# Haian-Jin/TensoIR

Hardware: AMD Instinct MI355X
Metric: primary+secondary rays/sec at 4096 rays x 512 samples (higher is better)
Workload: dtype f32 io and field; decoders split-bf16 x3 (hi/lo operands, 3 MFMA products), fp32 accumulate; indirect light (secondary-ray records): fp16 shadow taps + fp16 single-product decoder, fp32 accumulate

## Files before the change

tensoir_amd/csrc/tir_common.hpp:

```cpp
#pragma once
#include <hip/hip_runtime.h>
#include <stdint.h>
#include <initializer_list>
#include <type_traits>
#include "tensoir_hip.h"

#define TIR_WAVE 64

#define TIR_CHECK_LAUNCH()                                   \
    do {                                                     \
        hipError_t e__ = hipGetLastError();                  \
        if (e__ != hipSuccess) return -(int)e__;             \
    } while (0)

static inline hipStream_t tir_stream(void* s) { return reinterpret_cast<hipStream_t>(s); }

static inline int tir_xcd_mapping(const TirField* f) { return f->tune_xcd_order == 1 ? 1 : 0; }

#include <mutex>
#include <set>
#include <utility>
static inline int tir_allow_dynamic_lds(const void* kernel, int bytes) {
    static std::mutex mu;
    static std::set<std::pair<const void*, int>> done;
// ... 622 lines not shown
    }
    __builtin_amdgcn_wave_barrier();
    constexpr int PER = 64 / C4;
    const int slot_in = lane / C4, c = lane % C4;
    for (int base = 0; base < n; base += PER) {
        const int slot = base + slot_in;
        float part = 0.0f;
        if (slot < n) part = density_chunk_rec<C4>(f, ll, wr + slot * TIR_TAPREC, c);
        if (C4 >= 2) part += dpp_f<0xB1, 0xf>(0.0f, part);
        if (C4 >= 4) part += dpp_f<0x4E, 0xf>(0.0f, part);
        if (C4 >= 8) part += dpp_f<0x141, 0xf>(0.0f, part);
        if (slot < n && c == 0) wl[slot * TIR_TAPREC] = part;
    }
    __builtin_amdgcn_wave_barrier();
    float sig = 0.0f;
    if (valid) sig = feature2density(f, wl[rank * TIR_TAPREC]);
    __builtin_amdgcn_wave_barrier();
    return sig;
}

__device__ __forceinline__ float wave_sigma(const TirField& f, bool valid, float x, float y, float z, float* wl) {
    switch (f.n_dcomp) {
        case 16: return wave_sigma_t<4>(f, valid, x, y, z, wl);
        case 8:  return wave_sigma_t<2>(f, valid, x, y, z, wl);
        case 32: return wave_sigma_t<8>(f, valid, x, y, z, wl);
        default: return wave_sigma_t<1>(f, valid, x, y, z, wl);
    }
}

__device__ __forceinline__ float exp_neg_fast(float x) { return __builtin_amdgcn_exp2f(x * -1.4426950408889634f); }

__device__ __forceinline__ bool sample_valid(const TirField& f, float px, float py, float pz, float& x, float& y, float& z) {
    x = norm_coord(px, f.aabb_min[0], f.inv_aabb[0]);
    y = norm_coord(py, f.aabb_min[1], f.inv_aabb[1]);
    z = norm_coord(pz, f.aabb_min[2], f.inv_aabb[2]);
    if (!in_bbox(f, px, py, pz)) return false;
    if (f.occ_nbr != nullptr && !occupancy_hit(f, px, py, pz)) return false;
    return true;
}

__device__ __forceinline__ void occ_t_range(const float (&occ_lo)[3], const float (&occ_hi)[3], const float (&o)[3], const float (&d)[3],
                                            float& t0, float& t1) {
    t0 = -INFINITY; t1 = INFINITY;
    if (!((occ_lo[0] < occ_hi[0]) & (occ_lo[1] < occ_hi[1]) & (occ_lo[2] < occ_hi[2]))) return;
#pragma unroll
    for (int a = 0; a < 3; ++a) {
        if (fabsf(d[a]) < 1e-20f) {
            if ((o[a] < occ_lo[a]) | (o[a] > occ_hi[a])) { t0 = INFINITY; t1 = -INFINITY; }
        } else {
            const float inv = __builtin_amdgcn_rcpf(d[a]);
            const float ta = (occ_lo[a] - o[a]) * inv, tb = (occ_hi[a] - o[a]) * inv;
            t0 = fmaxf(t0, fminf(ta, tb));
            t1 = fminf(t1, fmaxf(ta, tb));
        }
    }
    t0 -= 1e-4f; t1 += 1e-4f;
}

struct UDiv { unsigned d, m; };
__device__ __forceinline__ UDiv make_udiv(int d) { return UDiv{d > 1 ? (unsigned)d : 1u, d > 1 ? 0xFFFFFFFFu / (unsigned)d : 0u}; }
__device__ __forceinline__ unsigned udiv(unsigned x, const UDiv& u, unsigned& rem) {
    if (u.d == 1) { rem = 0; return x; }
    unsigned q = __umulhi(x, u.m), r = x - q * u.d;
    if (r >= u.d) { q += 1; r -= u.d; }
    rem = r;
    return q;
}

__device__ __forceinline__ float linear2srgb(float x) {
    x = fminf(fmaxf(x, 0.0f), 1.0f);
    float lin = x * 12.92f;
    float nonlin = 1.055f * powf(x + 1e-6f, 0.41666666666666667f) - 0.055f;
    return (x <= 0.0031308f) ? lin : nonlin;
}

struct RaySetup {
    float o[3], d[3];
    float t_min;
};

__device__ __forceinline__ RaySetup ray_setup(const TirField& f, const float* __restrict__ rays, int r) {
    RaySetup s;
    float tm = -INFINITY;
#pragma unroll
    for (int a = 0; a < 3; ++a) {
        s.o[a] = rays[6 * (size_t)r + a];
        s.d[a] = rays[6 * (size_t)r + 3 + a];
        float vec = (s.d[a] == 0.0f) ? 1e-6f : s.d[a];
        float ra = __fdiv_rn(sub_rn(f.aabb_max[a], s.o[a]), vec);
        float rb = __fdiv_rn(sub_rn(f.aabb_min[a], s.o[a]), vec);
        tm = fmaxf(tm, fminf(ra, rb));
    }
    s.t_min = fminf(fmaxf(tm, f.near_), f.far_);
    return s;
}

__device__ __forceinline__ float sample_z(const TirField& f, float t_min, int k, float jitter, bool has_jitter) {
    float rng = (float)k;
    if (has_jitter) rng = add_rn(rng, jitter);
    return add_rn(t_min, mul_rn(f.step_size, rng));
}



__device__ __forceinline__ void philox_round(uint32_t (&c)[4], uint32_t k0, uint32_t k1) {
    const uint64_t p0 = (uint64_t)0xD2511F53u * c[0], p1 = (uint64_t)0xCD9E8D57u * c[2];
    const uint32_t n0 = (uint32_t)(p1 >> 32) ^ c[1] ^ k0, n2 = (uint32_t)(p0 >> 32) ^ c[3] ^ k1;
    c[0] = n0; c[1] = (uint32_t)p1; c[2] = n2; c[3] = (uint32_t)p0;
}

__device__ __forceinline__ void jitter_normals(unsigned long long seed, unsigned long long offset, uint64_t idx, float (&nrm)[3]) {
    uint32_t c[4] = {(uint32_t)idx, (uint32_t)(idx >> 32), (uint32_t)offset, (uint32_t)(offset >> 32)};
    uint32_t k0 = (uint32_t)seed, k1 = (uint32_t)(seed >> 32);
#pragma unroll
    for (int r = 0; r < 10; ++r) { philox_round(c, k0, k1); k0 += 0x9E3779B9u; k1 += 0xBB67AE85u; }
    const float u0 = ((float)c[0] + 0.5f) * 2.3283064365386963e-10f, u1 = ((float)c[1] + 0.5f) * 2.3283064365386963e-10f;
    const float u2 = ((float)c[2] + 0.5f) * 2.3283064365386963e-10f, u3 = ((float)c[3] + 0.5f) * 2.3283064365386963e-10f;
    const float r0 = sqrtf(-2.0f * logf(fminf(u0, 0.99999994f))), r1 = sqrtf(-2.0f * logf(fminf(u2, 0.99999994f)));
    float s0, c0, s1, c1;
    sincospif(2.0f * u1, &s0, &c0);
    sincospif(2.0f * u3, &s1, &c1);
    nrm[0] = r0 * c0; nrm[1] = r0 * s0; nrm[2] = r1 * c1;
    (void)s1;
}

__device__ __forceinline__ void philox_uniform4(unsigned long long seed, unsigned long long offset, uint64_t idx, float (&u)[4]) {
    uint32_t c[4] = {(uint32_t)idx, (uint32_t)(idx >> 32), (uint32_t)offset, (uint32_t)(offset >> 32)};
    uint32_t k0 = (uint32_t)seed, k1 = (uint32_t)(seed >> 32);
#pragma unroll
    for (int r = 0; r < 10; ++r) { philox_round(c, k0, k1); k0 += 0x9E3779B9u; k1 += 0xBB67AE85u; }
#pragma unroll
    for (int q = 0; q < 4; ++q) u[q] = fminf(((float)c[q] + 0.5f) * 2.3283064365386963e-10f, 0.99999994f);
}

struct XcdRange { long long first, end, stride; };
__device__ __forceinline__ XcdRange xcd_range_at(long long n_items, int per, bool on, int bid, int nblk) {
    XcdRange r;
    if (!on || (nblk & 7) != 0) {
        r.first = (long long)bid * per; r.end = n_items; r.stride = (long long)nblk * per;
        return r;
    }
    const int xcd = bid & 7, local = bid >> 3, per_xcd = nblk >> 3;
    const long long chunk = (n_items + 7) / 8;
    const long long lo = chunk * xcd;
    r.first = lo + (long long)local * per;
    r.end = lo + chunk < n_items ? lo + chunk : n_items;
    r.stride = (long long)per_xcd * per;
    return r;
}
__device__ __forceinline__ XcdRange xcd_range(long long n_items, int per, bool on) {
    return xcd_range_at(n_items, per, on, (int)blockIdx.x, (int)gridDim.x);
}

}
```

tensoir_amd/csrc/tir_march.hip:

```cpp
#include "tir_common.hpp"

using namespace tir;

__device__ __forceinline__ void march_one_ray(const TirField& f, const float* __restrict__ rays, const float* __restrict__ ray_jitter,
                                              int B, int S, float t_stop, float* __restrict__ weight, float* __restrict__ acc_out,
                                              float* __restrict__ depth_out, float* __restrict__ tend_out,
                                              int32_t* __restrict__ app_count, unsigned long long* __restrict__ stats,
                                              float* __restrict__ sigma_out, float* __restrict__ viewdirs, bool coh, int ray, int lane) {
    RaySetup rs = ray_setup(f, rays, ray);
    if (viewdirs && lane < 3) viewdirs[3 * (size_t)ray + lane] = rays[6 * (size_t)ray + 3 + lane];

    const bool hj = ray_jitter != nullptr;
    const float jit = hj ? ray_jitter[ray] : 0.0f;

    __shared__ __attribute__((aligned(16))) float wl_all[4][256];
    float* wl = wl_all[threadIdx.x >> 6];
    float T = 1.0f;
    float acc = 0.0f, depth = 0.0f;
    int cnt = 0;
    int k0 = 0;
    unsigned n_gather = 0;
    for (; k0 < S; k0 += 64) {
        const int k = k0 + lane;
        float z = 0.0f, x = 0.f, y = 0.f, zz = 0.f;
        bool valid = false;
        if (k < S) {
            z = sample_z(f, rs.t_min, k, jit, hj);
            float px = add_rn(rs.o[0], mul_rn(rs.d[0], z));
            float py = add_rn(rs.o[1], mul_rn(rs.d[1], z));
            float pz = add_rn(rs.o[2], mul_rn(rs.d[2], z));
            valid = sample_valid(f, px, py, pz, x, y, zz);
        }
        const float sigma = wave_sigma(f, valid, x, y, zz, wl);
        float w = 0.0f, v = 1.0f;
        if (k < S) {
            float dist = (k + 1 < S) ? sub_rn(sample_z(f, rs.t_min, k + 1, jit, hj), z) : 0.0f;
            float alpha = 1.0f - expf(-sigma * mul_rn(dist, f.distance_scale));
            v = add_rn(sub_rn(1.0f, alpha), 1e-10f);
            w = alpha;
        }
        float incl = scan_prod<64>(v, lane);
        float excl = shift_up1<64>(incl, lane);
        w = w * (T * excl);
        if (k < S) weight[(size_t)ray * S + k] = w;
        if (sigma_out && k < S) sigma_out[(size_t)ray * S + k] = sigma;
        acc += w;
        depth = fmaf(w, z, depth);
        cnt += __popcll(__ballot(w > f.weight_thres));
        if (stats) n_gather += __popcll(__ballot(valid));
        T = T * __shfl(incl, 63, 64);
        if (T < t_stop) { k0 += 64; break; }
    }
    for (; k0 < S; k0 += 64) {
        const int k = k0 + lane;
        if (k < S) weight[(size_t)ray * S + k] = 0.0f;
        if (sigma_out && k < S) sigma_out[(size_t)ray * S + k] = 0.0f;
    }
    acc = group_sum<64>(acc);
    depth = group_sum<64>(depth);
    if (lane == 0) {
        acc_out[ray] = acc;
        depth_out[ray] = depth;
        if (tend_out) tend_out[ray] = T;
        if (coh) __hip_atomic_store(app_count + ray, cnt, __ATOMIC_RELAXED, __HIP_MEMORY_SCOPE_AGENT);
        else app_count[ray] = cnt;
        if (stats) atomicAdd(stats, (unsigned long long)n_gather);
    }
}


struct TirMarchExtras {
    float* viewdirs;
    int32_t* zero_words; int n_zero;
    int32_t* ticket; int32_t* offsets; int cap; int32_t* total_out;
};

__device__ __forceinline__ void block_exclusive_scan_capped(const int32_t* __restrict__ counts, int32_t* __restrict__ offsets,
                                                             int n, int cap, int32_t* __restrict__ total_out) {
    __shared__ int32_t wsum[4];
    __shared__ int32_t carry_s;
    const int tid = threadIdx.x, lane = tid & 63, wv = tid >> 6;
    if (tid == 0) carry_s = 0;
    __syncthreads();
    for (int base = 0; base < n; base += 256) {
        const int i = base + tid;
        const int32_t v = (i < n) ? __hip_atomic_load(counts + i, __ATOMIC_RELAXED, __HIP_MEMORY_SCOPE_AGENT) : 0;
        int32_t incl = v;
#pragma unroll
        for (int d = 1; d < 64; d <<= 1) {
            int32_t o = __shfl_up(incl, d, 64);
            if (lane >= d) incl += o;
        }
        if (lane == 63) wsum[wv] = incl;
        __syncthreads();
        int32_t woff = 0;
        for (int q = 0; q < wv; ++q) woff += wsum[q];
        const int32_t carry = carry_s;
        if (i < n) offsets[i] = min(carry + woff + incl - v, cap);
        __syncthreads();
        if (tid == 255) carry_s = carry + woff + incl;
        __syncthreads();
    }
    if (tid == 0) {
        offsets[n] = min(carry_s, cap);
        if (total_out) *total_out = carry_s;
    }
}

__global__ void __launch_bounds__(256)
k_march_primary(TirField f, const float* __restrict__ rays, const float* __restrict__ ray_jitter,
                int B, int S, float t_stop, float* __restrict__ weight, float* __restrict__ acc_out,
                float* __restrict__ depth_out, float* __restrict__ tend_out, int32_t* __restrict__ app_count,
                unsigned long long* __restrict__ stats, float* __restrict__ sigma_out, TirMarchExtras ex) {
    const int lane = threadIdx.x & 63;
    const int ray = blockIdx.x * (blockDim.x >> 6) + (threadIdx.x >> 6);
    if (ex.zero_words && blockIdx.x == 0 && threadIdx.x < ex.n_zero) ex.zero_words[threadIdx.x] = 0;
    if (ray < B) march_one_ray(f, rays, ray_jitter, B, S, t_stop, weight, acc_out, depth_out, tend_out, app_count, stats,
                               sigma_out, ex.viewdirs, ex.ticket != nullptr, ray, lane);
    if (!ex.ticket) return;
    __shared__ int s_last;
    asm volatile("s_waitcnt vmcnt(0)" ::: "memory");
    __syncthreads();
    if (threadIdx.x == 0) {
        const int t = __hip_atomic_fetch_add(ex.ticket, 1, __ATOMIC_RELAXED, __HIP_MEMORY_SCOPE_AGENT);
        s_last = (t == (int)gridDim.x - 1);
        if (s_last) __hip_atomic_store(ex.ticket, 0, __ATOMIC_RELAXED, __HIP_MEMORY_SCOPE_AGENT);
    }
    __syncthreads();
    if (s_last) block_exclusive_scan_capped(app_count, ex.offsets, B, ex.cap, ex.total_out);
}

extern "C" int tir_march_primary_fwd(const TirField* f, const float* rays, const float* ray_jitter,
                                     int32_t B, int32_t S, float t_stop, float* weight, float* acc,
                                     float* depth, float* t_end, int32_t* app_count,
                                     unsigned long long* stats, void* stream) {
    if (!f || B < 0 || S <= 0) return TIR_ERR_ARG;
    if (B == 0) return TIR_OK;
    if (!rays || !weight || !acc || !depth || !app_count) return TIR_ERR_ARG;
    if (!(f->n_dcomp == 4 || f->n_dcomp == 8 || f->n_dcomp == 16 || f->n_dcomp == 32)) return TIR_ERR_UNSUPPORTED;
    if (!tir_occ_index_ok(f) || !tir_plane_index_ok(f)) return TIR_ERR_UNSUPPORTED;
    hipLaunchKernelGGL(k_march_primary, dim3((B + 3) / 4), dim3(256), 0, tir_stream(stream), *f, rays,
                       ray_jitter, B, S, t_stop, weight, acc, depth, t_end, app_count, stats, (float*)nullptr, TirMarchExtras{});
    TIR_CHECK_LAUNCH();
    return TIR_OK;
}

extern "C" int tir_march_primary_fused_fwd(const TirField* f, const float* rays, const float* ray_jitter,
                                           int32_t B, int32_t S, float t_stop, float* weight, float* acc,
                                           float* depth, float* t_end, int32_t* app_count, unsigned long long* stats,
                                           float* viewdirs, int32_t* zero_words, int32_t n_zero, int32_t* ticket,
                                           int32_t* offsets, int32_t cap, int32_t* total, void* stream) {
    if (!f || B < 0 || S <= 0 || n_zero < 0 || n_zero > 256 || cap < 0) return TIR_ERR_ARG;
    if ((ticket == nullptr) != (offsets == nullptr)) return TIR_ERR_ARG;
    if (B == 0) return TIR_OK;
    if (!rays || !weight || !acc || !depth || !app_count) return TIR_ERR_ARG;
    if (!(f->n_dcomp == 4 || f->n_dcomp == 8 || f->n_dcomp == 16 || f->n_dcomp == 32)) return TIR_ERR_UNSUPPORTED;
    if (!tir_occ_index_ok(f) || !tir_plane_index_ok(f)) return TIR_ERR_UNSUPPORTED;
    TirMarchExtras ex{viewdirs, zero_words, n_zero, ticket, offsets, cap, total};
    hipLaunchKernelGGL(k_march_primary, dim3((B + 3) / 4), dim3(256), 0, tir_stream(stream), *f, rays,
                       ray_jitter, B, S, t_stop, weight, acc, depth, t_end, app_count, stats, (float*)nullptr, ex);
    TIR_CHECK_LAUNCH();
    return TIR_OK;
}

extern "C" int tir_march_primary_train_fwd(const TirField* f, const float* rays, const float* ray_jitter,
                                           int32_t B, int32_t S, float t_stop, float* weight, float* sigma,
                                           float* acc, float* depth, float* t_end, int32_t* app_count, void* stream) {
    if (!f || B < 0 || S <= 0) return TIR_ERR_ARG;
    if (B == 0) return TIR_OK;
    if (!rays || !weight || !sigma || !acc || !depth || !app_count) return TIR_ERR_ARG;
    if (!(f->n_dcomp == 4 || f->n_dcomp == 8 || f->n_dcomp == 16 || f->n_dcomp == 32)) return TIR_ERR_UNSUPPORTED;
    if (!tir_occ_index_ok(f) || !tir_plane_index_ok(f)) return TIR_ERR_UNSUPPORTED;
    hipLaunchKernelGGL(k_march_primary, dim3((B + 3) / 4), dim3(256), 0, tir_stream(stream), *f, rays,
                       ray_jitter, B, S, t_stop, weight, acc, depth, t_end, app_count,
                       (unsigned long long*)nullptr, sigma, TirMarchExtras{});
    TIR_CHECK_LAUNCH();
    return TIR_OK;
}

__global__ void __launch_bounds__(1024)
k_exclusive_scan(const int32_t* __restrict__ counts, int32_t* __restrict__ offsets, int n, int cap,
                 int32_t* __restrict__ total_out) {
    __shared__ int32_t wsum[16];
    __shared__ int32_t carry_s;
    const int tid = threadIdx.x, lane = tid & 63, wv = tid >> 6;
    if (tid == 0) carry_s = 0;
    __syncthreads();
    for (int base = 0; base < n; base += 1024) {
        int i = base + tid;
        int32_t v = (i < n) ? counts[i] : 0;
        int32_t incl = v;
#pragma unroll
        for (int d = 1; d < 64; d <<= 1) {
            int32_t o = __shfl_up(incl, d, 64);
            if (lane >= d) incl += o;
        }
        if (lane == 63) wsum[wv] = incl;
        __syncthreads();
        int32_t woff = 0;
        for (int q = 0; q < wv; ++q) woff += wsum[q];
        int32_t carry = carry_s;
        if (i < n) offsets[i] = min(carry + woff + incl - v, cap);
        __syncthreads();
        if (tid == 1023) carry_s = carry + woff + incl;
        __syncthreads();
    }
    if (tid == 0) {
        offsets[n] = min(carry_s, cap);
        if (total_out) *total_out = carry_s;
    }
}

extern "C" int tir_exclusive_scan(const int32_t* counts, int32_t* offsets, int32_t n, void* stream) {
    if (!offsets || n < 0 || (n > 0 && !counts)) return TIR_ERR_ARG;
    hipLaunchKernelGGL(k_exclusive_scan, dim3(1), dim3(1024), 0, tir_stream(stream), counts, offsets, n, 0x7fffffff,
                       (int32_t*)nullptr);
    TIR_CHECK_LAUNCH();
    return TIR_OK;
}

extern "C" int tir_exclusive_scan_capped(const int32_t* counts, int32_t* offsets, int32_t n, int32_t cap,
                                         int32_t* total, void* stream) {
    if (!offsets || n < 0 || cap < 0 || (n > 0 && !counts)) return TIR_ERR_ARG;
    hipLaunchKernelGGL(k_exclusive_scan, dim3(1), dim3(1024), 0, tir_stream(stream), counts, offsets, n, cap, total);
    TIR_CHECK_LAUNCH();
    return TIR_OK;
}

struct TirCheck4 { const int32_t* cnt[4]; int64_t cap[4]; int n; };

__global__ void k_record_check(TirCheck4 c, int64_t* __restrict__ state, int64_t* __restrict__ host_out) {
    if (threadIdx.x != 0 || blockIdx.x != 0) return;
    int64_t over = state[4];
    for (int i = 0; i < 4; ++i) {
        int64_t v = 0;
        if (i < c.n) {
            v = *c.cnt[i];
            if (v > c.cap[i]) over = 1;
            if (v > state[i]) state[i] = v;
        }
        host_out[i] = v;
        host_out[4 + i] = state[i];
    }
    state[4] = over;
    host_out[8] = over;
    __threadfence_system();
}

extern "C" int tir_record_check(const int32_t* const* counters, const int64_t* caps, int32_t n, int64_t* state,
                                int64_t* host_out, void* stream) {
    if (n < 0 || n > 4 || !state || !host_out || (n > 0 && (!counters || !caps))) return TIR_ERR_ARG;
// ... 581 lines not shown
        }
        __syncthreads();
        int32_t* const rec_ray = s_park.rec_ray;
        float* const rec_w = s_park.rec_w;
        float* const rec_xyz = s_park.rec_xyz;
#pragma unroll
        for (int g = 0; g < 4; ++g) {
            const int rl = g * NHW + hw;
            int base = s_base[rl];
            if (base < 0) continue;
            const int64_t ray = s_pid[rl];
            const float4 s0 = *reinterpret_cast<const float4*>(sh + 24 * g);
            const float2 s1 = *reinterpret_cast<const float2*>(sh + 24 * g + 4);
            const float o[3] = {s0.x, s0.y, s0.z}, d[3] = {s0.w, s1.x, s1.y};
#pragma unroll
            for (int st = 0; st < NSTEP; ++st) {
                const int k = st * 32 + hl;
                const float w = wreg[REC ? g : 0][REC ? st : 0];
                const bool keep = w > f.weight_thres;
                const unsigned hm = (unsigned)(__ballot(keep) >> half_shift);
                if (keep) {
                    const int slot = base + __popc(hm & ((1u << hl) - 1u));
                    const float z = zt[k];
                    rec_ray[slot] = (int32_t)ray;
                    rec_w[slot] = w;
#pragma unroll
                    for (int a = 0; a < 3; ++a) {
                        float p = add_rn(o[a], mul_rn(d[a], z));
                        rec_xyz[3 * (size_t)slot + a] = norm_coord(p, f.aabb_min[a], f.inv_aabb[a]);
                    }
                }
                base += __popc(hm);
            }
        }
    }
    if (stats && hl == 0 && n_gather) atomicAdd(s_park.stats, (unsigned long long)n_gather);
}

#define TIR_SEC_KERNEL_PARAMS                                                                                                  \
    TirField f, const float* __restrict__ origins, const int32_t* __restrict__ org_map, const float* __restrict__ dirs,       \
    const int32_t* __restrict__ dir_map, const uint8_t* __restrict__ active, int64_t n_rays, int n_dirs, int n_sample,        \
    const float* __restrict__ z_vals, float t_stop, float* __restrict__ vis, float* __restrict__ one_minus_acc,               \
    int32_t* __restrict__ rec_counter, int64_t rec_cap, int32_t* __restrict__ rec_ray, float* __restrict__ rec_w,             \
    float* __restrict__ rec_xyz, int32_t* __restrict__ ray_rec_off, int32_t* __restrict__ ray_rec_cnt,                        \
    unsigned long long* __restrict__ stats, int xcd_on, const int32_t* __restrict__ ray_ids, const int32_t* __restrict__ n_ids_dev
#define TIR_SEC_KERNEL_ARGS                                                                                                    \
    f, origins, org_map, dirs, dir_map, active, n_rays, n_dirs, n_sample, z_vals, t_stop, vis, one_minus_acc, rec_counter,    \
    rec_cap, rec_ray, rec_w, rec_xyz, ray_rec_off, ray_rec_cnt, stats, xcd_on, ray_ids, n_ids_dev

template <int C4, int NSTEP, int NT, bool REC>
__global__ void __launch_bounds__(NT, 4)
k_march_secondary_lds(TIR_SEC_KERNEL_PARAMS, int line_floats) {
    march_secondary_body<C4, NSTEP, NT, REC, false>(TIR_SEC_KERNEL_ARGS, line_floats);
}

#define TIR_DENSE_WAVES 6
template <int NSTEP, bool REC>
__global__ void __launch_bounds__(512, TIR_DENSE_WAVES)
k_march_secondary_dense(TIR_SEC_KERNEL_PARAMS) {
    march_secondary_body<1, NSTEP, 512, REC, true>(TIR_SEC_KERNEL_ARGS, 0);
}


extern "C" int tir_march_secondary_fwd(const TirField* f, const float* origins, const int32_t* org_map,
                                       const float* dirs, const int32_t* dir_map, const uint8_t* active,
                                       int64_t n_rays, int32_t n_dirs, int32_t n_sample, const float* z_vals,
                                       float t_stop, float* vis, float* one_minus_acc,
                                       int32_t* rec_counter, int64_t rec_cap, int32_t* rec_ray,
                                       float* rec_w, float* rec_xyz, int32_t* ray_rec_off,
                                       int32_t* ray_rec_cnt, unsigned long long* stats, void* stream) {
    return tir_march_secondary_ids_fwd(f, origins, org_map, dirs, dir_map, active, n_rays, n_dirs, n_sample, z_vals, t_stop,
                                       vis, one_minus_acc, rec_counter, rec_cap, rec_ray, rec_w, rec_xyz, ray_rec_off,
                                       ray_rec_cnt, stats, nullptr, nullptr, stream);
}

extern "C" int tir_march_secondary_ids_fwd(const TirField* f, const float* origins, const int32_t* org_map,
                                           const float* dirs, const int32_t* dir_map, const uint8_t* active,
                                           int64_t n_rays, int32_t n_dirs, int32_t n_sample, const float* z_vals,
                                           float t_stop, float* vis, float* one_minus_acc,
                                           int32_t* rec_counter, int64_t rec_cap, int32_t* rec_ray,
                                           float* rec_w, float* rec_xyz, int32_t* ray_rec_off,
                                           int32_t* ray_rec_cnt, unsigned long long* stats, const int32_t* ray_ids,
                                           const int32_t* n_ids_dev, void* stream) {
    if (!f || n_rays < 0 || n_sample <= 0) return TIR_ERR_ARG;
    if ((ray_ids == nullptr) != (n_ids_dev == nullptr)) return TIR_ERR_ARG;
    if (n_sample > TIR_SEC_MAX_SAMPLES) return TIR_ERR_UNSUPPORTED;
    if (n_rays == 0) return TIR_OK;
    if (!origins || !dirs || !z_vals) return TIR_ERR_ARG;
    if (rec_counter && (!rec_ray || !rec_w || !rec_xyz || !ray_rec_off || !ray_rec_cnt || rec_cap < 0)) return TIR_ERR_ARG;
    if (n_rays >= (int64_t)1 << 31) return TIR_ERR_UNSUPPORTED;
    if (!(f->n_dcomp == 4 || f->n_dcomp == 8 || f->n_dcomp == 16 || f->n_dcomp == 32)) return TIR_ERR_UNSUPPORTED;
    if (!tir_occ_index_ok(f) || !tir_plane_index_ok(f)) return TIR_ERR_UNSUPPORTED;
    const int xcd_on = tir_xcd_mapping(f);
    if (tir_dense_sigma_ok(f) && (n_sample <= 96 || !rec_counter)) {
        const int64_t n_batches = (n_rays + 63) / 64;
        unsigned nblk = (unsigned)std::min<int64_t>(n_batches, (TIR_DENSE_WAVES / 2) * 256);
        if (xcd_on) nblk = (nblk + 7) / 8 * 8;
        const size_t lds = ((size_t)((n_sample + 3) & ~3) + 3 * 64) * sizeof(float);
#define TIR_LAUNCH_SEC_DENSE(NSTEP_, REC_)                                                                                  \
        hipLaunchKernelGGL((k_march_secondary_dense<NSTEP_, REC_>), dim3(nblk), dim3(512), lds, tir_stream(stream), *f,     \
                           origins, org_map, dirs, dir_map, active, n_rays, n_dirs, n_sample, z_vals, t_stop, vis,          \
                           one_minus_acc, rec_counter, rec_cap, rec_ray, rec_w, rec_xyz, ray_rec_off, ray_rec_cnt, stats,   \
                           xcd_on, ray_ids, n_ids_dev)
        if (rec_counter) TIR_LAUNCH_SEC_DENSE(3, true);
        else if (n_sample <= 96) TIR_LAUNCH_SEC_DENSE(3, false);
        else TIR_LAUNCH_SEC_DENSE(8, false);
#undef TIR_LAUNCH_SEC_DENSE
        TIR_CHECK_LAUNCH();
        return TIR_OK;
    }
    {
        const int64_t line_floats = (int64_t)(f->grid[0] + f->grid[1] + f->grid[2]) * f->n_dcomp;
        const size_t fixed = ((size_t)line_floats + ((n_sample + 3) & ~3)) * sizeof(float);
        const size_t lds512 = fixed + (8 * 64 * TIR_TAPREC + 3 * 64) * sizeof(float), lds1024 = fixed + (16 * 64 * TIR_TAPREC + 3 * 128) * sizeof(float);
        if (f->tune_lds_lines != 2 && f->n_dcomp == 16 && n_sample <= 96 && f->grid[0] < 65536 && f->grid[1] < 65536 && f->grid[2] < 65536 && lds1024 + 8192 <= 158 * 1024) {
            const bool small = lds512 + 4096 <= 80 * 1024;
            const int rpb = small ? 64 : 128;
            const int64_t n_batches = (n_rays + rpb - 1) / rpb;
            unsigned nblk = (unsigned)std::min<int64_t>(n_batches, small ? 2 * 256 : 256);
            if (xcd_on) nblk = (nblk + 7) / 8 * 8;
#define TIR_LAUNCH_SEC_LDS(NT_, REC_, LDS_, CAP_)                                                                                          \
            do {                                                                                                                          \
                if (int rc = tir_allow_dynamic_lds(reinterpret_cast<const void*>(k_march_secondary_lds<4, 3, NT_, REC_>), CAP_)) return rc; \
                hipLaunchKernelGGL((k_march_secondary_lds<4, 3, NT_, REC_>), dim3(nblk), dim3(NT_), LDS_, tir_stream(stream),             \
                                   *f, origins, org_map, dirs, dir_map, active, n_rays, n_dirs, n_sample, z_vals, t_stop, vis,            \
                                   one_minus_acc, rec_counter, rec_cap, rec_ray, rec_w, rec_xyz, ray_rec_off, ray_rec_cnt, stats,         \
                                   xcd_on, ray_ids, n_ids_dev, (int)line_floats);                                                         \
            } while (0)
            if (small) { if (rec_counter) TIR_LAUNCH_SEC_LDS(512, true, lds512, 80 * 1024); else TIR_LAUNCH_SEC_LDS(512, false, lds512, 80 * 1024); }
            else       { if (rec_counter) TIR_LAUNCH_SEC_LDS(1024, true, lds1024, 150 * 1024); else TIR_LAUNCH_SEC_LDS(1024, false, lds1024, 150 * 1024); }
#undef TIR_LAUNCH_SEC_LDS
            TIR_CHECK_LAUNCH();
            return TIR_OK;
        }
    }
    size_t lds = ((size_t)((n_sample + 3) & ~3) + 4 * 256 + 4 * TIR_SEC_RPB +
                  (rec_counter ? (size_t)TIR_SEC_RPB * n_sample : 0)) * sizeof(float);
    unsigned nblk = (unsigned)((n_rays + TIR_SEC_RPB - 1) / TIR_SEC_RPB);
    if (xcd_on) nblk = (nblk + 7) / 8 * 8;
    hipLaunchKernelGGL(k_march_secondary, dim3(nblk), dim3(256), lds, tir_stream(stream),
                       *f, origins, org_map, dirs, dir_map, active, n_rays, n_dirs, n_sample, z_vals, t_stop, vis,
                       one_minus_acc, rec_counter, rec_cap, rec_ray, rec_w, rec_xyz, ray_rec_off, ray_rec_cnt, stats, xcd_on,
                       ray_ids, n_ids_dev);
    TIR_CHECK_LAUNCH();
    return TIR_OK;
}

__global__ void __launch_bounds__(256)
k_accumulate_records(const int32_t* __restrict__ off, const int32_t* __restrict__ cnt,
                     const float* __restrict__ rec_w, const float* __restrict__ rec_rgb, int64_t n,
                     float* __restrict__ indirect) {
    int64_t p = (int64_t)blockIdx.x * blockDim.x + threadIdx.x;
    if (p >= n) return;
    float c0 = 0, c1 = 0, c2 = 0;
    const int b = off[p], e = b + cnt[p];
    for (int i = b; i < e; ++i) {
        float w = rec_w[i];
        c0 = fmaf(w, rec_rgb[3 * (size_t)i], c0);
        c1 = fmaf(w, rec_rgb[3 * (size_t)i + 1], c1);
        c2 = fmaf(w, rec_rgb[3 * (size_t)i + 2], c2);
    }
    indirect[3 * p] = c0; indirect[3 * p + 1] = c1; indirect[3 * p + 2] = c2;
}

extern "C" int tir_accumulate_records(const int32_t* ray_rec_off, const int32_t* ray_rec_cnt,
                                      const float* rec_w, const float* rec_rgb, int64_t n_rays,
                                      float* indirect, void* stream) {
    if (n_rays < 0) return TIR_ERR_ARG;
    if (n_rays == 0) return TIR_OK;
    if (!ray_rec_off || !ray_rec_cnt || !indirect) return TIR_ERR_ARG;
    hipLaunchKernelGGL(k_accumulate_records, dim3((unsigned)((n_rays + 255) / 256)), dim3(256), 0,
                       tir_stream(stream), ray_rec_off, ray_rec_cnt, rec_w, rec_rgb, n_rays, indirect);
    TIR_CHECK_LAUNCH();
    return TIR_OK;
}
```

tensoir_amd/csrc/tir_shade.hip:

```cpp
#include "tir_common.hpp"

using namespace tir;

namespace {

__device__ __forceinline__ void normalize3(float& x, float& y, float& z, float eps) {
    float n = fmaxf(sqrtf(x * x + y * y + z * z), eps);
    x /= n; y /= n; z /= n;
}

struct Surface {
    float N[3], V[3];
    float NoV;
    float alpha2[3], k[3];
    float fres[3];
    float alb_pi[3];
};

__device__ __forceinline__ Surface make_surface(const float* normal, const float* view, const float* rough3,
                                                const float* fres3, const float* albedo) {
    Surface s;
    s.N[0] = normal[0]; s.N[1] = normal[1]; s.N[2] = normal[2];
    s.V[0] = view[0]; s.V[1] = view[1]; s.V[2] = view[2];
    normalize3(s.V[0], s.V[1], s.V[2], 1e-12f);
    normalize3(s.N[0], s.N[1], s.N[2], 1e-12f);
    float nov = s.V[0] * s.N[0] + s.V[1] * s.N[1] + s.V[2] * s.N[2];
    float sg = (nov > 0.f) ? 1.f : ((nov < 0.f) ? -1.f : 0.f);
    s.N[0] *= sg; s.N[1] *= sg; s.N[2] *= sg;
    nov = s.N[0] * s.V[0] + s.N[1] * s.V[1] + s.N[2] * s.V[2];
    s.NoV = fminf(fmaxf(nov, 1e-6f), 1.f);
#pragma unroll
    for (int c = 0; c < 3; ++c) {
        float r = rough3[c];
        float a = r * r;
        s.alpha2[c] = a * a;
        s.k[c] = (a + 2.f * r + 1.0f) / 8.0f;
        s.fres[c] = fres3[c];
        s.alb_pi[c] = albedo ? albedo[c] / 3.14159265358979323846f : 0.f;
    }
    return s;
}

__device__ __forceinline__ void ggx_dir(const Surface& s, float lx, float ly, float lz, float spec[3]) {
    normalize3(lx, ly, lz, 1e-12f);
    float hx = (lx + s.V[0]) / 2.0f, hy = (ly + s.V[1]) / 2.0f, hz = (lz + s.V[2]) / 2.0f;
    normalize3(hx, hy, hz, 1e-12f);
    float NoL = fminf(fmaxf(s.N[0] * lx + s.N[1] * ly + s.N[2] * lz, 1e-6f), 1.f);
    float NoH = fminf(fmaxf(s.N[0] * hx + s.N[1] * hy + s.N[2] * hz, 1e-6f), 1.f);
    float VoH = fminf(fmaxf(s.V[0] * hx + s.V[1] * hy + s.V[2] * hz, 1e-6f), 1.f);
    float FMi = ((-5.55473f) * VoH - 6.98316f) * VoH;
    float p2 = exp2f(FMi);
    const float four_pi = 4.0f * 3.14159265358979323846f;
#pragma unroll
    for (int c = 0; c < 3; ++c) {
        float frac0 = s.fres[c] + (1.f - s.fres[c]) * p2;
        float frac = frac0 * s.alpha2[c];
        float nom0 = NoH * NoH * (s.alpha2[c] - 1.f) + 1.f;
        float nom1 = s.NoV * (1.f - s.k[c]) + s.k[c];
        float nom2 = NoL * (1.f - s.k[c]) + s.k[c];
        float nom = fminf(fmaxf(four_pi * nom0 * nom0 * nom1 * nom2, 1e-6f), four_pi);
        spec[c] = frac / nom;
    }
}

__global__ void __launch_bounds__(128)
k_env_sg(TirEnvSG e, const float* __restrict__ dirs, int D, float* __restrict__ out) {
    const int ld = blockIdx.x;
    const int l = ld / D, d = ld % D;
    const float v0 = dirs[3 * d], v1 = dirs[3 * d + 1], v2 = dirs[3 * d + 2];
    const float* R = e.rot + 9 * l;
    const float r0 = v0 * R[0] + v1 * R[3] + v2 * R[6];
    const float r1 = v0 * R[1] + v1 * R[4] + v2 * R[7];
    const float r2 = v0 * R[2] + v1 * R[5] + v2 * R[8];
    float c0 = 0.f, c1 = 0.f, c2 = 0.f;
    for (int k = threadIdx.x; k < e.n_sg; k += blockDim.x) {
        const float* g = e.sgs + 7 * k;
        float nrm = sqrtf(g[0] * g[0] + g[1] * g[1] + g[2] * g[2]);
        float dot = r0 * (g[0] / nrm) + r1 * (g[1] / nrm) + r2 * (g[2] / nrm);
        float ex = expf(fabsf(g[3]) * (dot - 1.0f));
        c0 += fabsf(g[4]) * ex; c1 += fabsf(g[5]) * ex; c2 += fabsf(g[6]) * ex;
    }
    __shared__ float red[3][2];
    c0 = group_sum<64>(c0); c1 = group_sum<64>(c1); c2 = group_sum<64>(c2);
    const int wv = threadIdx.x >> 6;
    if ((threadIdx.x & 63) == 0) { red[0][wv] = c0; red[1][wv] = c1; red[2][wv] = c2; }
    __syncthreads();
    if (threadIdx.x == 0) {
        float* o = out + 3 * (size_t)ld;
        o[0] = red[0][0] + red[0][1]; o[1] = red[1][0] + red[1][1]; o[2] = red[2][0] + red[2][1];
    }
}

__global__ void __launch_bounds__(1024)
k_shade_setup(const float* __restrict__ maps, const float* __restrict__ rays, const float* __restrict__ dirs,
              int M, int D, float acc_thres, float* __restrict__ surf, uint8_t* __restrict__ active,
              int32_t* __restrict__ pair_ids, int32_t* __restrict__ n_active, float* __restrict__ vis,
              int32_t* __restrict__ rec_cnt, int dir_major) {
    const int64_t t = (int64_t)blockIdx.x * blockDim.x + threadIdx.x;
    const bool in = t < (int64_t)M * D;
    int64_t i = t;
    if (dir_major && in) i = (t % M) * D + t / M;
    bool act = false;
    if (in) {
        const int m = (int)(i / D), d = (int)(i % D);
        const float* mp = maps + (size_t)m * TIR_MAP_STRIDE;
        const float* r = rays + 6 * (size_t)m;
        if (d == 0) {
            const float depth = mp[3];
#pragma unroll
            for (int a = 0; a < 3; ++a) surf[3 * (size_t)m + a] = add_rn(r[a], mul_rn(depth, r[3 + a]));
        }
        float cs = dirs[3 * d] * mp[4] + dirs[3 * d + 1] * mp[5] + dirs[3 * d + 2] * mp[6];
        act = fmaxf(cs, 0.f) > 1e-6f && mp[14] > acc_thres;
        active[i] = act ? 1 : 0;
    }
    if (!pair_ids) return;
    __shared__ int s_wcnt[16];
    __shared__ int s_base;
    const unsigned long long mask = __ballot(act);
    const int lane = threadIdx.x & 63, wv = threadIdx.x >> 6, nw = blockDim.x >> 6;
    if (lane == 0) s_wcnt[wv] = __popcll(mask);
    __syncthreads();
    if (threadIdx.x == 0) {
        int tot = 0;
        for (int q = 0; q < nw; ++q) { const int c = s_wcnt[q]; s_wcnt[q] = tot; tot += c; }
        s_base = tot ? atomicAdd(n_active, tot) : 0;
    }
    __syncthreads();
    const int base = s_base + s_wcnt[wv];
    if (act) {
        const int64_t slot = (int64_t)base + __popcll(mask & ((1ull << lane) - 1ull));
        if (slot < (int64_t)M * D) pair_ids[slot] = (int32_t)i;
    } else if (in) {
        if (vis) vis[i] = 0.0f;
        if (rec_cnt) rec_cnt[i] = 0;
    }
}

__global__ void __launch_bounds__(256)
k_shade_integrate(const float* __restrict__ maps, const float* __restrict__ rays, const float* __restrict__ dirs,
                  const int32_t* __restrict__ light_idx, const float* __restrict__ vis,
                  const float* __restrict__ indirect, const float* __restrict__ env,
                  const float* __restrict__ weight_d, int M, int D, int n_lights, int equal_area, int use_srgb,
                  float acc_thres, float* __restrict__ out, const int32_t* __restrict__ rec_off,
                  const int32_t* __restrict__ rec_cnt, const float* __restrict__ rec_w, const float* __restrict__ rec_rgb,
                  int32_t* __restrict__ reset_counter) {
    const int lane = threadIdx.x & 63;
    if (reset_counter && blockIdx.x == 0 && threadIdx.x == 0) *reset_counter = 0;
    const int m = blockIdx.x * (blockDim.x >> 6) + (threadIdx.x >> 6);
    if (m >= M) return;
    const float* mp = maps + (size_t)m * TIR_MAP_STRIDE;
    if (!(mp[14] > acc_thres)) {
        if (lane < 3) out[3 * (size_t)m + lane] = 1.0f;
        return;
    }
    const float* r = rays + 6 * (size_t)m;
    float view[3] = {-r[3], -r[4], -r[5]};
    normalize3(view[0], view[1], view[2], 1e-6f);
    const float rough3[3] = {mp[10], mp[10], mp[10]};
    Surface s = make_surface(mp + 4, view, rough3, mp + 11, mp + 7);
    int li = light_idx ? light_idx[m] : 0;
    li = min(max(li, 0), n_lights - 1);
    const float* envl = env + (size_t)li * D * 3;
    float c[3] = {0.f, 0.f, 0.f};
    for (int d = lane; d < D; d += 64) {
        const float lx = dirs[3 * d], ly = dirs[3 * d + 1], lz = dirs[3 * d + 2];
        const float cosine = fmaxf(lx * mp[4] + ly * mp[5] + lz * mp[6], 0.f);
        float spec[3];
        ggx_dir(s, lx, ly, lz, spec);
        const size_t md = (size_t)m * D + d;
        const float v = vis[md];
        const float wd = equal_area ? 1.0f : weight_d[d];
        float ind[3] = {0.f, 0.f, 0.f};
        if (indirect) { ind[0] = indirect[3 * md]; ind[1] = indirect[3 * md + 1]; ind[2] = indirect[3 * md + 2]; }
        else if (rec_off) {
            const int b = rec_off[md], e = b + rec_cnt[md];
            for (int i = b; i < e; ++i) {
                const float w = rec_w[i];
                ind[0] = fmaf(w, rec_rgb[3 * (size_t)i], ind[0]);
                ind[1] = fmaf(w, rec_rgb[3 * (size_t)i + 1], ind[1]);
                ind[2] = fmaf(w, rec_rgb[3 * (size_t)i + 2], ind[2]);
            }
        }
#pragma unroll
        for (int q = 0; q < 3; ++q) {
            float light = v * envl[3 * d + q] + ind[q];
            float brdf = s.alb_pi[q] + spec[q];
            if (equal_area) c[q] += 4.0f * 3.14159265358979323846f * brdf * light * cosine;
            else c[q] += brdf * light * cosine * wd;
        }
    }
#pragma unroll
    for (int q = 0; q < 3; ++q) {
        float t = group_sum<64>(c[q]);
        if (equal_area) t /= (float)D;
        t = fminf(fmaxf(t, 0.f), 1.f);
        if (use_srgb) t = linear2srgb(t);
        if (lane == 0) out[3 * (size_t)m + q] = t;
    }
}

__global__ void __launch_bounds__(256)
k_relight_importance(const float* __restrict__ normal, const float* __restrict__ albedo,
                     const float* __restrict__ rough, const float* __restrict__ fresnel,
                     const float* __restrict__ rays_d, const float* __restrict__ ldir,
                     const float* __restrict__ lrgb, const float* __restrict__ lpdf,
                     const float* __restrict__ vis, int M, int Ns, float* __restrict__ out) {
    const int lane = threadIdx.x & 63;
    const int m = blockIdx.x * (blockDim.x >> 6) + (threadIdx.x >> 6);
    if (m >= M) return;
    float view[3] = {-rays_d[3 * (size_t)m], -rays_d[3 * (size_t)m + 1], -rays_d[3 * (size_t)m + 2]};
    normalize3(view[0], view[1], view[2], 1e-6f);
    const float rough3[3] = {rough[m], rough[m], rough[m]};
    const float* nm = normal + 3 * (size_t)m;
    Surface s = make_surface(nm, view, rough3, fresnel + 3 * (size_t)m, albedo + 3 * (size_t)m);
    float c[3] = {0.f, 0.f, 0.f};
    for (int j = lane; j < Ns; j += 64) {
        const size_t mj = (size_t)m * Ns + j;
        const float lx = ldir[3 * mj], ly = ldir[3 * mj + 1], lz = ldir[3 * mj + 2];
        const float cosine = lx * nm[0] + ly * nm[1] + lz * nm[2];
        float spec[3];
        ggx_dir(s, lx, ly, lz, spec);
        const float v = vis[mj], pdf = lpdf[mj];
#pragma unroll
        for (int q = 0; q < 3; ++q)
            c[q] += (s.alb_pi[q] + spec[q]) * (v * lrgb[3 * mj + q]) * cosine / pdf;
    }
#pragma unroll
    for (int q = 0; q < 3; ++q) {
        float t = group_sum<64>(c[q]) / (float)Ns;
        t = linear2srgb(fminf(fmaxf(t, 0.f), 1.f));
        if (lane == 0) out[3 * (size_t)m + q] = t;
    }
}

__device__ __forceinline__ int cdf_upper_bound(const float* __restrict__ cdf, int n, float u) {
    int lo = 0, hi = n - 1;
    while (lo < hi) {
        const int mid = (lo + hi) >> 1;
        if (cdf[mid] > u) hi = mid; else lo = mid + 1;
    }
    return lo;
}

template <typename G>
__device__ __forceinline__ int cdf_upper_bound_guided(const float* __restrict__ cdf, int n, float u, const G* __restrict__ guide, int g) {
    const int k = min((int)(u * (float)g), g - 1);
    int lo = (int)guide[k], hi = (int)guide[k + 1];
    while (lo < hi) {
        const int mid = (lo + hi) >> 1;
        if (cdf[mid] > u) hi = mid; else lo = mid + 1;
    }
    return lo;
}

__global__ void __launch_bounds__(256)
k_env_sample_setup(const float* __restrict__ row_cdf, const float* __restrict__ col_cdf, int H, int W,
                   const float* __restrict__ env_dir, const float* __restrict__ normal, int M, int Ns,
                   unsigned long long seed, unsigned long long offset, int32_t* __restrict__ cell,
                   uint8_t* __restrict__ active) {
    const int64_t i = (int64_t)blockIdx.x * blockDim.x + threadIdx.x;
    if (i >= (int64_t)M * Ns) return;
    const int m = (int)(i / Ns);
    float u[4];
    tir::philox_uniform4(seed, offset, (uint64_t)i, u);
    const int row = cdf_upper_bound(row_cdf, H, u[0]);
    const int col = cdf_upper_bound(col_cdf + (size_t)row * W, W, u[1]);
    const int c = row * W + col;
    cell[i] = c;
    const float* d = env_dir + 3 * (size_t)c;
    const float* nm = normal + 3 * (size_t)m;
    const float cosine = d[0] * nm[0] + d[1] * nm[1] + d[2] * nm[2];
    active[i] = cosine > 1e-6f ? 1 : 0;
}

__global__ void __launch_bounds__(256)
k_env_sample_list(const float* __restrict__ row_cdf, const float* __restrict__ col_cdf, int H, int W,
                    const float* __restrict__ env_dir, int dir_stride, const float* __restrict__ normal, int M, int Ns,
                    unsigned long long seed, unsigned long long offset, int bins_r, int bins_c, int block_pairs,
                    const int32_t* __restrict__ row_guide, const uint16_t* __restrict__ col_guide, int g_rows, int g_cols,
                    int32_t* __restrict__ cell, float* __restrict__ vis, int32_t* __restrict__ pair_ids,
                    int32_t* __restrict__ n_active, const int32_t* __restrict__ m_dev) {
    extern __shared__ __attribute__((aligned(16))) unsigned char sb_lds[];
    if (m_dev) M = min(M, max(*m_dev, 0));
    uint16_t* const list = reinterpret_cast<uint16_t*>(sb_lds);
    uint8_t* const keys = sb_lds + (size_t)block_pairs * 2;
    __shared__ int s_hist[256], s_cursor[256], s_base;
    const int64_t n = (int64_t)M * Ns;
    const int64_t base = (int64_t)blockIdx.x * block_pairs;
    if (base >= n) return;
    const int cnt = (int)min((int64_t)block_pairs, n - base);
    const int n_bins = bins_r * bins_c;
    s_hist[threadIdx.x] = 0;
    __syncthreads();
    for (int j = threadIdx.x; j < cnt; j += 256) {
        const int64_t i = base + j;
        const int m = (int)(i / Ns);
        float u[4];
        tir::philox_uniform4(seed, offset, (uint64_t)i, u);
        const int row = row_guide ? cdf_upper_bound_guided(row_cdf, H, u[0], row_guide, g_rows) : cdf_upper_bound(row_cdf, H, u[0]);
        const int col = col_guide ? cdf_upper_bound_guided(col_cdf + (size_t)row * W, W, u[1], col_guide + (size_t)row * (g_cols + 2), g_cols)
                                  : cdf_upper_bound(col_cdf + (size_t)row * W, W, u[1]);
        const int c = row * W + col;
        cell[i] = c;
        const float* d = env_dir + (size_t)dir_stride * (size_t)c;
        const float* nm = normal + 3 * (size_t)m;
        const float cosine = d[0] * nm[0] + d[1] * nm[1] + d[2] * nm[2];
        int key = 255;
        if (cosine > 1e-6f) {
            key = (int)(((int64_t)row * bins_r) / H) * bins_c + (int)(((int64_t)col * bins_c) / W);
            atomicAdd(&s_hist[key], 1);
        } else {
            vis[i] = 0.0f;
        }
        keys[j] = (uint8_t)key;
    }
    __syncthreads();
    {
        const int lane = threadIdx.x & 63, wv = threadIdx.x >> 6;
        const int c = s_hist[threadIdx.x];
        int incl = c;
#pragma unroll
        for (int dd = 1; dd < 64; dd <<= 1) {
            const int oth = __shfl_up(incl, dd, 64);
            if (lane >= dd) incl += oth;
        }
        __shared__ int s_wsum[4];
        if (lane == 63) s_wsum[wv] = incl;
        __syncthreads();
        int before = 0;
        for (int q = 0; q < wv; ++q) before += s_wsum[q];
        s_cursor[threadIdx.x] = before + incl - c;
        if (threadIdx.x == 255) {
            const int total = before + incl;
            s_hist[0] = total;
            s_base = total > 0 ? atomicAdd(n_active, total) : 0;
        }
    }
    __syncthreads();
    for (int j = threadIdx.x; j < cnt; j += 256) {
        const int key = keys[j];
        if (key < n_bins) list[atomicAdd(&s_cursor[key], 1)] = (uint16_t)j;
// ... 620 lines not shown
```

Baseline: 5.285 million.

## Batch record loads, unroll shade direction loop, and widen per-thread scan

Adds a grouped record-sum helper that issues loads for eight records before the FMAs, so each record walk has more loads in flight. The shade-integrate loop now handles two directions per lane and prefetches their direction, env, vis and record offset data before computing, with a launch-bounds occupancy hint. The block exclusive scan now has each thread scan sixteen consecutive counts serially, which cuts the number of barrier iterations. The costs are higher register pressure and clamped redundant loads in the tail.

```diff
diff --git a/tensoir_amd/csrc/tir_common.hpp b/tensoir_amd/csrc/tir_common.hpp
--- a/tensoir_amd/csrc/tir_common.hpp
+++ b/tensoir_amd/csrc/tir_common.hpp
@@ -798,4 +798,37 @@
     return xcd_range_at(n_items, per, on, (int)blockIdx.x, (int)gridDim.x);
 }
 
-}
+template <int G>
+__device__ __forceinline__ void record_sum(const float* __restrict__ rec_w, const float* __restrict__ rec_rgb, int b, int e,
+                                           float (&acc)[3]) {
+    int i = b;
+    for (; e - i >= G; i += G) {
+        float w[G], c[G][3];
+#pragma unroll
+        for (int j = 0; j < G; ++j) {
+            w[j] = rec_w[i + j];
+            c[j][0] = rec_rgb[3 * (size_t)(i + j)]; c[j][1] = rec_rgb[3 * (size_t)(i + j) + 1]; c[j][2] = rec_rgb[3 * (size_t)(i + j) + 2];
+        }
+#pragma unroll
+        for (int j = 0; j < G; ++j) {
+            acc[0] = fmaf(w[j], c[j][0], acc[0]); acc[1] = fmaf(w[j], c[j][1], acc[1]); acc[2] = fmaf(w[j], c[j][2], acc[2]);
+        }
+    }
+    if (i < e) {
+        float w[G - 1], c[G - 1][3];
+#pragma unroll
+        for (int j = 0; j < G - 1; ++j) {
+            const size_t k = (size_t)min(i + j, e - 1);
+            w[j] = rec_w[k];
+            c[j][0] = rec_rgb[3 * k]; c[j][1] = rec_rgb[3 * k + 1]; c[j][2] = rec_rgb[3 * k + 2];
+        }
+#pragma unroll
+        for (int j = 0; j < G - 1; ++j)
+            if (i + j < e) {
+                acc[0] = fmaf(w[j], c[j][0], acc[0]); acc[1] = fmaf(w[j], c[j][1], acc[1]); acc[2] = fmaf(w[j], c[j][2], acc[2]);
+            }
+    }
+}
+constexpr int RECORD_GROUP = 8;
+
+}
diff --git a/tensoir_amd/csrc/tir_march.hip b/tensoir_amd/csrc/tir_march.hip
--- a/tensoir_amd/csrc/tir_march.hip
+++ b/tensoir_amd/csrc/tir_march.hip
@@ -77,15 +77,26 @@
 
 __device__ __forceinline__ void block_exclusive_scan_capped(const int32_t* __restrict__ counts, int32_t* __restrict__ offsets,
                                                              int n, int cap, int32_t* __restrict__ total_out) {
+    constexpr int SCAN_PER = 16;
     __shared__ int32_t wsum[4];
     __shared__ int32_t carry_s;
     const int tid = threadIdx.x, lane = tid & 63, wv = tid >> 6;
     if (tid == 0) carry_s = 0;
     __syncthreads();
-    for (int base = 0; base < n; base += 256) {
-        const int i = base + tid;
-        const int32_t v = (i < n) ? __hip_atomic_load(counts + i, __ATOMIC_RELAXED, __HIP_MEMORY_SCOPE_AGENT) : 0;
-        int32_t incl = v;
+    for (int base = 0; base < n; base += 256 * SCAN_PER) {
+        const int i0 = base + SCAN_PER * tid;
+        int32_t v[SCAN_PER];
+#pragma unroll
+        for (int j = 0; j < SCAN_PER; ++j)
+            v[j] = __hip_atomic_load(counts + min(i0 + j, n - 1), __ATOMIC_RELAXED, __HIP_MEMORY_SCOPE_AGENT);
+        int32_t sum = 0;
+#pragma unroll
+        for (int j = 0; j < SCAN_PER; ++j) {
+            const int32_t x = (i0 + j < n) ? v[j] : 0;
+            v[j] = sum;
+            sum += x;
+        }
+        int32_t incl = sum;
 #pragma unroll
         for (int d = 1; d < 64; d <<= 1) {
             int32_t o = __shfl_up(incl, d, 64);
@@ -96,7 +107,10 @@
         int32_t woff = 0;
         for (int q = 0; q < wv; ++q) woff += wsum[q];
         const int32_t carry = carry_s;
-        if (i < n) offsets[i] = min(carry + woff + incl - v, cap);
+        const int32_t first = carry + woff + incl - sum;
+#pragma unroll
+        for (int j = 0; j < SCAN_PER; ++j)
+            if (i0 + j < n) offsets[i0 + j] = min(first + v[j], cap);
         __syncthreads();
         if (tid == 255) carry_s = carry + woff + incl;
         __syncthreads();
@@ -984,15 +998,10 @@
                      float* __restrict__ indirect) {
     int64_t p = (int64_t)blockIdx.x * blockDim.x + threadIdx.x;
     if (p >= n) return;
-    float c0 = 0, c1 = 0, c2 = 0;
+    float c[3] = {0.f, 0.f, 0.f};
     const int b = off[p], e = b + cnt[p];
-    for (int i = b; i < e; ++i) {
-        float w = rec_w[i];
-        c0 = fmaf(w, rec_rgb[3 * (size_t)i], c0);
-        c1 = fmaf(w, rec_rgb[3 * (size_t)i + 1], c1);
-        c2 = fmaf(w, rec_rgb[3 * (size_t)i + 2], c2);
-    }
-    indirect[3 * p] = c0; indirect[3 * p + 1] = c1; indirect[3 * p + 2] = c2;
+    record_sum<RECORD_GROUP>(rec_w, rec_rgb, b, e, c);
+    indirect[3 * p] = c[0]; indirect[3 * p + 1] = c[1]; indirect[3 * p + 2] = c[2];
 }
 
 extern "C" int tir_accumulate_records(const int32_t* ray_rec_off, const int32_t* ray_rec_cnt,
diff --git a/tensoir_amd/csrc/tir_shade.hip b/tensoir_amd/csrc/tir_shade.hip
--- a/tensoir_amd/csrc/tir_shade.hip
+++ b/tensoir_amd/csrc/tir_shade.hip
@@ -137,7 +137,7 @@
     }
 }
 
-__global__ void __launch_bounds__(256)
+__global__ void __launch_bounds__(256, 4)
 k_shade_integrate(const float* __restrict__ maps, const float* __restrict__ rays, const float* __restrict__ dirs,
                   const int32_t* __restrict__ light_idx, const float* __restrict__ vis,
                   const float* __restrict__ indirect, const float* __restrict__ env,
@@ -163,31 +163,41 @@
     li = min(max(li, 0), n_lights - 1);
     const float* envl = env + (size_t)li * D * 3;
     float c[3] = {0.f, 0.f, 0.f};
-    for (int d = lane; d < D; d += 64) {
-        const float lx = dirs[3 * d], ly = dirs[3 * d + 1], lz = dirs[3 * d + 2];
-        const float cosine = fmaxf(lx * mp[4] + ly * mp[5] + lz * mp[6], 0.f);
-        float spec[3];
-        ggx_dir(s, lx, ly, lz, spec);
-        const size_t md = (size_t)m * D + d;
-        const float v = vis[md];
-        const float wd = equal_area ? 1.0f : weight_d[d];
-        float ind[3] = {0.f, 0.f, 0.f};
-        if (indirect) { ind[0] = indirect[3 * md]; ind[1] = indirect[3 * md + 1]; ind[2] = indirect[3 * md + 2]; }
-        else if (rec_off) {
-            const int b = rec_off[md], e = b + rec_cnt[md];
-            for (int i = b; i < e; ++i) {
-                const float w = rec_w[i];
-                ind[0] = fmaf(w, rec_rgb[3 * (size_t)i], ind[0]);
-                ind[1] = fmaf(w, rec_rgb[3 * (size_t)i + 1], ind[1]);
-                ind[2] = fmaf(w, rec_rgb[3 * (size_t)i + 2], ind[2]);
+    const bool from_records = !indirect && rec_off;
+    for (int d0 = lane; d0 < D; d0 += 128) {
+        const bool two = d0 + 64 < D;
+        float l2[2][3], e2[2][3], w2[2], v2[2];
+        int b2[2] = {0, 0}, n2[2] = {0, 0};
+#pragma unroll
+        for (int u = 0; u < 2; ++u) {
+            const int d = (u && two) ? d0 + 64 : d0;
+            const size_t md = (size_t)m * D + d;
+#pragma unroll
+            for (int q = 0; q < 3; ++q) { l2[u][q] = dirs[3 * d + q]; e2[u][q] = envl[3 * d + q]; }
+            w2[u] = equal_area ? 1.0f : weight_d[d];
+            v2[u] = vis[md];
+            if (from_records) { b2[u] = rec_off[md]; n2[u] = rec_cnt[md]; }
+        }
+#pragma unroll
+        for (int u = 0; u < 2; ++u) {
+            if (u && !two) break;
+            const float lx = l2[u][0], ly = l2[u][1], lz = l2[u][2];
+            const float cosine = fmaxf(lx * mp[4] + ly * mp[5] + lz * mp[6], 0.f);
+            float spec[3];
+            ggx_dir(s, lx, ly, lz, spec);
+            const size_t md = (size_t)m * D + d0 + 64 * u;
+            const float v = v2[u];
+            const float wd = w2[u];
+            float ind[3] = {0.f, 0.f, 0.f};
+            if (indirect) { ind[0] = indirect[3 * md]; ind[1] = indirect[3 * md + 1]; ind[2] = indirect[3 * md + 2]; }
+            else if (rec_off) record_sum<RECORD_GROUP>(rec_w, rec_rgb, b2[u], b2[u] + n2[u], ind);
+#pragma unroll
+            for (int q = 0; q < 3; ++q) {
+                float light = v * e2[u][q] + ind[q];
+                float brdf = s.alb_pi[q] + spec[q];
+                if (equal_area) c[q] += 4.0f * 3.14159265358979323846f * brdf * light * cosine;
+                else c[q] += brdf * light * cosine * wd;
             }
-        }
-#pragma unroll
-        for (int q = 0; q < 3; ++q) {
-            float light = v * envl[3 * d + q] + ind[q];
-            float brdf = s.alb_pi[q] + spec[q];
-            if (equal_area) c[q] += 4.0f * 3.14159265358979323846f * brdf * light * cosine;
-            else c[q] += brdf * light * cosine * wd;
         }
     }
 #pragma unroll
```

Result: faster. 5.406 million (median of 6 runs) (+2.3%).
